# matuszelenak/Hybrid-Genome-Assembler

Hardware: AMD Instinct MI355X
Metric: k-mers/s counted + reads/s categorized, k=19 E.coli 30×; %HBM roofline (higher is better)
Workload: dtype u64; 1 GPU; C2: k=19 count of an E. coli-sized pair (4.64 + 5.07 Mb, d=0.021), ART-like 30x 150 bp, 2 files; per step: count_run + spec_hist + select[10,25]; k=19, reads=1941478, bases=293163176, instances_per_gpu=256275096, distinct_rows=6680801, selected=1820729, discriminative=1820245, buckets=4096, max_split=1, parallelism=dp1

## Files before the change

### hybrid-genome-assembler_amd/csrc/api.hip

```cpp
#include <cstdlib>
#include <cstring>
#include <string>
#include <type_traits>
#include <vector>

#include "hga_internal.hpp"

namespace {
thread_local std::string g_err;

template <class F>
hga_status guard(F&& f) {
    static_assert(std::is_void<decltype(f())>::value, "guarded bodies return nothing");
    try {
        g_err.clear();
        f();
        return HGA_OK;
    } catch (const hga::Error& e) {
        g_err = e.what();
        return e.code;
    } catch (const std::bad_alloc&) {
        g_err = "host allocation failed";
        return HGA_ERR_OOM;
    } catch (const std::exception& e) {
// ... 51 lines not shown
        HGA_REQUIRE(device >= 0 && device < nd, HGA_ERR_INVALID, "no such HIP device");
        HGA_HIP(hipSetDevice(device));
        auto* c = new hga_ctx();
        c->device = device;
        hipDeviceProp_t prop;
        if (hipGetDeviceProperties(&prop, device) == hipSuccess && prop.multiProcessorCount > 0)
            c->num_cu = prop.multiProcessorCount;
        hipError_t e = hipStreamCreateWithFlags(&c->stream, hipStreamNonBlocking);
        if (e != hipSuccess) {
            delete c;
            throw hga::Error(HGA_ERR_HIP, std::string("hipStreamCreate: ") + hipGetErrorString(e));
        }
        *out = c;
    });
}

hga_status hga_ctx_destroy(hga_ctx* c) {
    if (!c) return HGA_OK;
    return guard([&] {
        (void)hipSetDevice(c->device);
        (void)hipStreamSynchronize(c->stream);
        if (c->side) (void)hipStreamSynchronize(c->side);
        hipStream_t s = c->stream, s2 = c->side;
        hipEvent_t e1 = c->ev_fork, e2 = c->ev_join;
        delete c;
        (void)hipStreamDestroy(s);
        if (s2) {
            (void)hipEventDestroy(e1);
            (void)hipEventDestroy(e2);
            (void)hipStreamDestroy(s2);
        }
    });
}

hga_status hga_count_begin(hga_ctx* c, int k, uint32_t n_files) {
    HGA_CTX_GUARD(c, hga::count_begin(c, k, n_files));
}

hga_status hga_count_add(hga_ctx* c, uint32_t file, const char* seq, uint64_t n_bytes) {
    HGA_CTX_GUARD(c, {
        HGA_REQUIRE(seq || n_bytes == 0, HGA_ERR_INVALID, "null sequence pointer");
        hga::count_add(c, file, seq, n_bytes);
    });
}

hga_status hga_connections_run(hga_ctx* c, const uint32_t* pivots, uint64_t n_pivots, uint32_t min_kmers,
                               uint64_t min_score, const int32_t* categories, uint64_t* n) {
    HGA_CTX_GUARD(c, {
// ... 384 lines not shown
```

### hybrid-genome-assembler_amd/csrc/count.hip

```cpp
#include <algorithm>
#include <cstdlib>
#include <cstring>
#include <map>
#include <type_traits>

#include "hga_internal.hpp"
#include "kmer_dev.hpp"

#ifndef HGA_B1_NOFB
#define HGA_B1_NOFB 0
#endif
#ifndef HGA_B1_BRANCHFREE
#define HGA_B1_BRANCHFREE 0
#endif

namespace hga {
namespace {

constexpr int NT_B = 512;
constexpr int P_B = 16;
constexpr int TP_B = NT_B * P_B;
constexpr uint64_t ST_ALIGN = TP_B;
#ifndef HGA_MAX_FB
#define HGA_MAX_FB 12
// ... 561 lines not shown
    }
    __syncthreads();
#pragma unroll
    for (int j = 0; j < IT; ++j) {
        const uint32_t i = (uint32_t)j * NT_R + tid;
        if (i < used) stage[off2[dd[j]] + rk[j]] = ee[j];
    }
    __syncthreads();
    for (uint32_t d = (uint32_t)__builtin_amdgcn_readfirstlane(tid >> 6); d < nb2; d += NT_R / 64) {
        const uint32_t o = off2[d], len = off2[d + 1] - o;
        E* __restrict__ dst = out + base2[d];
        for (uint32_t jj = (uint32_t)(tid & 63); jj < len; jj += 64) {
            if (HGA_NT_REBIN_ST) __builtin_nontemporal_store(stage[o + jj], &dst[jj]);
            else dst[jj] = stage[o + jj];
        }
    }
}

template <class E1, class E>
__global__ void __launch_bounds__(NT_R_MAX) kc_rebin(const E1* __restrict__ in1, const Blk* __restrict__ table,
                                                 const unsigned long long* __restrict__ gstat, uint32_t W,
                                                 KP kp, const uint32_t* __restrict__ nblk,
                                                 unsigned long long* __restrict__ off,
                                                 E* __restrict__ out, bool first) {
    if (first) {
        rebin_block<E1, E>(blockIdx.x, in1, table, W, kp, nblk, off, out);
        return;
    }
    const uint64_t n_first = (uint64_t)W * kp.nb1, used = gstat[3];
    for (uint64_t blk = n_first + blockIdx.x; blk < used; blk += gridDim.x) {
        rebin_block<E1, E>(blk, in1, table, W, kp, nblk, off, out);
        __syncthreads();
    }
}

#ifndef HGA_GROUP
#define HGA_GROUP 4
#endif
constexpr int GRP = HGA_GROUP;
template <class E>
__device__ __forceinline__ void read_group(const E* keys, uint32_t g, E (&k)[GRP]) {
    if constexpr (sizeof(E) == 4) {
#pragma unroll
        for (int t = 0; t < GRP / 4; ++t) {
            const uint4 v = reinterpret_cast<const uint4*>(keys)[g * (GRP / 4) + t];
            k[4 * t] = v.x; k[4 * t + 1] = v.y; k[4 * t + 2] = v.z; k[4 * t + 3] = v.w;
        }
    } else {
#pragma unroll
        for (int t = 0; t < GRP / 2; ++t) {
            const ulonglong2 a = reinterpret_cast<const ulonglong2*>(keys)[g * (GRP / 2) + t];
            k[2 * t] = a.x; k[2 * t + 1] = a.y;
        }
// ... 1117 lines not shown
    };
    if (lo > hi) {
        if (t < 4) span[t] = 0;
        publish(0u);
        return;
    }
    uint32_t lg = 0;
    while ((hi >> lg) - (lo >> lg) + 1 > 256) ++lg;
    const uint32_t dbase = lo >> lg;
    uint32_t sum = 0;
    const uint32_t b0 = (dbase + t) << lg;
    for (uint32_t b = b0; b < b0 + (1u << lg); ++b)
        if (b >= lo && b <= hi) sum += hist[b];
    if (t == 0) {
        span[0] = lo;
        span[1] = hi;
        span[2] = lg;
        span[3] = dbase;
    }
    publish(sum);
}

constexpr uint32_t BX_MAX = 1024;
__global__ void __launch_bounds__(1024) kc_bx_prep(const uint32_t* __restrict__ hist, const unsigned long long* __restrict__ wcnt,
                                                   uint32_t grid, uint32_t* __restrict__ dbase,
                                                   unsigned long long* __restrict__ stat,
                                                   unsigned long long* __restrict__ hstat) {
    __shared__ uint32_t ws[1024 / 64 + 1];
    __shared__ unsigned long long red[3][16];
    const uint32_t t = threadIdx.x, lane = t & 63, wave = t >> 6;
    uint32_t h[4], sum = 0, mx = 0;
#pragma unroll
    for (int q = 0; q < 4; ++q) {
        h[q] = hist[4 * t + q];
        sum += h[q];
        mx = max(mx, h[q]);
    }
    uint32_t tot;
    uint32_t o = block_excl_scan<1024>(sum, ws, &tot);
#pragma unroll
    for (int q = 0; q < 4; ++q) {
        dbase[4 * t + q] = o;
        o += h[q];
    }
    unsigned long long k = 0, d = 0, m = mx;
    for (uint32_t i = t; i < grid; i += 1024) {
        k += wcnt[2 * i];
        d += wcnt[2 * i + 1];
    }
#pragma unroll
    for (int s2 = 32; s2; s2 >>= 1) {
        k += __shfl_xor(k, s2, 64);
        d += __shfl_xor(d, s2, 64);
        m = max(m, (unsigned long long)__shfl_xor(m, s2, 64));
    }
    if (lane == 0) {
        red[0][wave] = k;
        red[1][wave] = d;
        red[2][wave] = m;
    }
    __syncthreads();
    if (t < 4) {
        unsigned long long v = 0;
        for (int w = 0; w < 16; ++w) v = t == 2 ? max(v, red[2][w]) : v + (t < 2 ? red[t][w] : 0ull);
        stat[t] = v;
        hstat[t] = v;
    }
}
__global__ void __launch_bounds__(256) kc_bx_colscan(const uint32_t* __restrict__ rows, uint32_t n_rows,
                                                     const uint32_t* __restrict__ dbase, uint32_t* __restrict__ off) {
    __shared__ uint32_t part[16][17];
    const uint32_t dl = threadIdx.x & 15, rg = threadIdx.x >> 4, d = blockIdx.x * 16 + dl;
    const uint32_t per = (n_rows + 15) / 16, r0 = rg * per, r1 = min(n_rows, r0 + per);
    uint32_t s2 = 0;
    for (uint32_t r = r0; r < r1; ++r) s2 += rows[(uint64_t)r * SEL_HB + d];
    part[rg][dl] = s2;
    __syncthreads();
    uint32_t base = dbase[d];
    for (uint32_t g = 0; g < rg; ++g) base += part[g][dl];
    for (uint32_t r = r0; r < r1; ++r) {
        off[(uint64_t)r * SEL_HB + d] = base;
        base += rows[(uint64_t)r * SEL_HB + d];
    }
}
__global__ void __launch_bounds__(256) kc_bx_scatter(const uint64_t* __restrict__ wkeys, uint64_t region,
                                                     const unsigned long long* __restrict__ wcnt,
                                                     const uint32_t* __restrict__ off, int hshift,
                                                     uint64_t* __restrict__ out) {
    __shared__ uint32_t cur[SEL_HB];
    const uint32_t w = blockIdx.x;
    for (uint32_t i = threadIdx.x; i < SEL_HB; i += 256) cur[i] = off[(uint64_t)w * SEL_HB + i];
    __syncthreads();
    const uint64_t n = wcnt[2 * w];
    const uint64_t* __restrict__ src = wkeys + (uint64_t)w * region;
    for (uint64_t j = threadIdx.x; j < n; j += 256) {
        const uint64_t key = src[j];
        const uint32_t pos = atomicAdd(&cur[(uint32_t)(key >> hshift) & (SEL_HB - 1)], 1u);
        out[pos] = key;
    }
}
template <int R>
__device__ __forceinline__ void bx_sort_seg(uint64_t* __restrict__ keys, uint32_t start, uint32_t len, uint32_t lane,
                                            int bits) {
    const uint64_t cm = bits >= 63 ? ~0ull >> 1 : (1ull << bits) - 1;
    uint64_t v[R];
#pragma unroll
    for (int u = 0; u < R; ++u) {
        const uint32_t i = lane * R + u;
        const uint64_t k = i < len ? keys[start + i] : 0ull;
        v[u] = i < len ? ((k & cm) << 1) | (k >> 63) : ~0ull;
    }
    bitonic_stage<R, 2>(v, lane);
// ... 4 lines not shown
    }
}
template <int R>
__device__ __forceinline__ void bx_sort_seg32(uint64_t* __restrict__ keys, uint32_t start, uint32_t len, uint32_t lane,
                                              int bits, uint64_t dig) {
    const int lb = bits - 12;
    const uint64_t lm = (1ull << lb) - 1;
    uint32_t v[R];
#pragma unroll
    for (int u = 0; u < R; ++u) {
        const uint32_t i = lane * R + u;
        const uint64_t k = i < len ? keys[start + i] : 0ull;
        v[u] = i < len ? (uint32_t)(((k & lm) << 1) | (k >> 63)) : ~0u;
    }
    bitonic_stage<R, 2>(v, lane);
    const uint64_t hi = dig << lb;
#pragma unroll
    for (int u = 0; u < R; ++u) {
        const uint32_t i = lane * R + u;
        if (i < len) keys[start + i] = hi | (uint64_t)(v[u] >> 1) | ((uint64_t)(v[u] & 1u) << 63);
    }
}
__global__ void __launch_bounds__(256) kc_bx_wsort(uint64_t* __restrict__ keys, const uint32_t* __restrict__ hist,
                                                   const uint32_t* __restrict__ dbase, int bits) {
    const uint32_t d = blockIdx.x * 4 + (threadIdx.x >> 6), lane = threadIdx.x & 63;
    const uint32_t len = hist[d], st = dbase[d];
    if (len <= 1 || len > BX_MAX) return;
    if (bits - 12 + 1 <= 32) {
        if (len <= 64) bx_sort_seg32<1>(keys, st, len, lane, bits, d);
        else if (len <= 256) bx_sort_seg32<4>(keys, st, len, lane, bits, d);
        else if (len <= 512) bx_sort_seg32<8>(keys, st, len, lane, bits, d);
        else bx_sort_seg32<16>(keys, st, len, lane, bits, d);
        return;
    }
    if (len <= 64) bx_sort_seg<1>(keys, st, len, lane, bits);
    else if (len <= 256) bx_sort_seg<4>(keys, st, len, lane, bits);
    else if (len <= 512) bx_sort_seg<8>(keys, st, len, lane, bits);
    else bx_sort_seg<16>(keys, st, len, lane, bits);
}

constexpr uint32_t BX_CAP32 = SS_T * 2 * SS_I;
template <bool U32, int NT, int I, int DB>
__global__ void __launch_bounds__(NT) kc_bx_lsort(uint64_t* __restrict__ keys, const uint32_t* __restrict__ hist,
                                                  const uint32_t* __restrict__ dbase, int bits, uint32_t min_len) {
    using T = std::conditional_t<U32, uint32_t, uint64_t>;
    __shared__ T sk[NT * I];
    __shared__ uint32_t wcnt[NT / 64][1 << DB];
// ... 195 lines not shown

    uint64_t st_pos = total_bytes / ((uint64_t)c->num_cu * HGA_B1_PER_CU) + 1;
    const uint64_t st_cap = (uint64_t)BLK * nb1 * 15 / 16;
    const char* sole_env = std::getenv("HGA_B1_SOLE");
    if ((!sole_env || std::atoi(sole_env) != 0) && st_pos > st_cap + st_cap / 2) st_pos = st_cap;
    st_pos = std::max<uint64_t>(ST_ALIGN, (st_pos + ST_ALIGN - 1) / ST_ALIGN * ST_ALIGN);
    std::vector<uint32_t> n_st(F, 0);
    std::vector<BinFile> bf(F);
    uint32_t W = 0;
    for (uint32_t f = 0; f < F; ++f) {
        n_st[f] = (uint32_t)((s.seq_len[f] + st_pos - 1) / st_pos);
        bf[f].n = s.seq_len[f];
        bf[f].w0 = W;
        W += n_st[f];
    }

    auto* gstat = static_cast<unsigned long long*>(s.cursor.ensure(8 * 8));
    uint64_t* fs = static_cast<uint64_t*>(s.file_start.ensure((size_t)nb * (F + 1) * 8));
    uint32_t* wcnt = static_cast<uint32_t*>(s.fine_hist.ensure((size_t)std::max<uint32_t>(W, 1) * nb * 4));
    auto* off = static_cast<unsigned long long*>(s.cursor2.ensure(((size_t)W * nb + 1) * 8));
    uint32_t* nblk = static_cast<uint32_t*>(s.nblk.ensure((size_t)std::max<uint32_t>(W, 1) * nb1 * 4));
    for (uint32_t f = 0; f < F; ++f) bf[f].seq = s.seq[f]->as<uint8_t>();
    const size_t tb = sizeof(BinFile) * F;
    std::vector<char> tab(tb);
    std::memcpy(tab.data(), bf.data(), tb);
    char* d_tab = static_cast<char*>(s.bin_files.ensure(tb));
    if (s.tab_host != tab) {
        HGA_HIP(hipMemcpy(d_tab, tab.data(), tb, hipMemcpyHostToDevice));
        s.tab_host = tab;
    }
    BinFile* d_bf = reinterpret_cast<BinFile*>(d_tab);

    const size_t esz1 = e1_32 ? 4 : 8, esz = e32 ? 4 : 8;
    uint64_t cap = (total_bytes / std::max<uint32_t>(1, min_per_file) + 4) & ~3ull;
    if (const char* e = std::getenv("HGA_ROW_CAP")) cap = std::max<uint64_t>(4, std::strtoull(e, nullptr, 10) & ~3ull);
    const uint32_t slot_b = (uint32_t)esz + 4u * F;
    uint32_t T = 1;
    while ((uint64_t)T * 2 * slot_b <= LDS_TAB) T *= 2;
    HGA_REQUIRE(T >= 2 * NT_C, HGA_ERR_INVALID, "too many files for the LDS table");
    const uint32_t maxload = std::min<uint32_t>((uint32_t)(T * 0.85), T - NT_C - 8);
    void* binned = s.binned.ensure(std::max<size_t>(total_bytes, 1) * esz);

    const uint64_t n_first = (uint64_t)W * nb1;
    const uint64_t table_cap = n_first + total_bytes / BLK + 2;
    const uint64_t pool_cap = table_cap * BLK;
    void* binned1 = s.binned1.ensure(pool_cap * esz1);
    Blk* table = static_cast<Blk*>(s.regions.ensure(table_cap * sizeof(Blk)));
    c->launch("kc_init", [&] { hipLaunchKernelGGL(kc_init_stat, dim3(1), dim3(64), 0, c->stream, gstat, n_first); });
    c->check_launch("kc_init");

    if (W) {
        c->launch("kc_bin1", [&] {
#define HGA_BIN1(E1T, KK, FBB)                                                                              \
    hipLaunchKernelGGL((kc_bin1<E1T, KK, FBB>), dim3(W), dim3(NT_B), 0, c->stream, d_bf, F, st_pos, kp, table, table_cap, \
                       pool_cap, static_cast<E1T*>(binned1), wcnt, nblk, gstat)
            if (e1_32 && kp.k == 19 && kp.fb == MAX_FB && !HGA_B1_NOFB) HGA_BIN1(uint32_t, 19, MAX_FB);
            else if (e1_32 && kp.k == 19) HGA_BIN1(uint32_t, 19, 0);
            else if (e1_32 && kp.k == 17) HGA_BIN1(uint32_t, 17, 0);
            else if (e1_32 && kp.k == 15) HGA_BIN1(uint32_t, 15, 0);
            else if (e1_32) HGA_BIN1(uint32_t, 0, 0);
            else if (kp.k == 21) HGA_BIN1(uint64_t, 21, 0);
            else HGA_BIN1(uint64_t, 0, 0);
#undef HGA_BIN1
        });
        c->check_launch("kc_bin1");
    }
    c->launch("kc_layout", [&] {
        hipLaunchKernelGGL(kc_transpose, dim3(blocks_for(nb, 64), blocks_for(std::max<uint32_t>(W, 1), 64)), dim3(256),
                           0, c->stream, wcnt, W, nb, reinterpret_cast<uint64_t*>(off));
    });
    c->check_launch("kc_transpose");
    exclusive_scan_u64(c, reinterpret_cast<uint64_t*>(off), (uint64_t)W * nb + 1, s.scratch);
    c->launch("kc_layout", [&] {
        hipLaunchKernelGGL(kc_fs, dim3(blocks_for((uint64_t)nb * (F + 1), 256)), dim3(256), 0, c->stream,
                           reinterpret_cast<const uint64_t*>(off), d_bf, W, nb, F, fs);
    });
    c->check_launch("kc_fs");
    const unsigned spill_grid = (unsigned)std::min<uint64_t>(table_cap - n_first, HGA_SPILL_GRID);
    c->launch("kc_rebin", [&] {
#define HGA_REBIN(E1T, ET)                                                                                 \
    do {                                                                                                   \
        if (n_first)                                                                                       \
            hipLaunchKernelGGL((kc_rebin<E1T, ET>), dim3((unsigned)n_first), dim3(rebin_nt<ET>()), 0, c->stream, \
                               static_cast<const E1T*>(binned1), table, gstat, W, kp, nblk, off,            \
                               static_cast<ET*>(binned), true);                                              \
        if (spill_grid)                                                                                    \
            hipLaunchKernelGGL((kc_rebin<E1T, ET>), dim3(spill_grid), dim3(rebin_nt<ET>()), 0, c->stream,  \
                               static_cast<const E1T*>(binned1), table, gstat, W, kp, nblk, off,            \
                               static_cast<ET*>(binned), false);                                             \
    } while (0)
        if (e1_32 && e32) HGA_REBIN(uint32_t, uint32_t);
        else if (e32) HGA_REBIN(uint64_t, uint32_t);
        else if (e1_32) HGA_REBIN(uint32_t, uint64_t);
        else HGA_REBIN(uint64_t, uint64_t);
#undef HGA_REBIN
    });
    c->check_launch("kc_rebin");
    uint32_t fb3 = 0;
    {
        const uint64_t avg = total_bytes >> fb;
        const char* te = std::getenv("HGA_SPLIT3_TARGET");
        const char* fe = std::getenv("HGA_SPLIT3_FORCE");
        const uint64_t target = te ? std::strtoull(te, nullptr, 10) : 32768;
        if (fe) {
            const uint32_t want = (uint32_t)std::atoi(fe);
            while (fb3 < want && fb3 < 8 && ((2u << fb3) * F) <= MAX_SF3 && kp.rbits - fb3 > 1) ++fb3;
        } else if (avg > 2 * per_bucket && fb == MAX_FB) {
            while (fb3 < 8 && (avg >> fb3) > target && ((2u << fb3) * F) <= MAX_SF3 && kp.rbits - fb3 > 10) ++fb3;
        }
    }
    if (fb3) {
        const uint32_t S = 1u << fb3;
        void* binned3 = s.binned3.ensure((total_bytes + total_bytes / 4 + (uint64_t)nb * S * SLACK_3 + 64) * esz);
// ... 222 lines not shown
    const bool use_bnd = n_thr <= 8 && !std::getenv("HGA_SPEC_FP64");
    if (fresh || s.thr_dev != thr) {
        HGA_HIP(hipMemcpyAsync(dthr, hthr, n_thr * 8, hipMemcpyHostToDevice, c->stream));
        if (n_thr <= 8) {
            std::vector<uint16_t> b((size_t)TL * 8, 0xFFFF);
            for (uint32_t t = 1; t < TL; ++t)
                for (uint32_t i = 0; i < n_thr; ++i) {
                    uint32_t lo = 0, hi = t + 1;
                    while (lo < hi) {
                        const uint32_t mid = (lo + hi) / 2;
                        const volatile double x = (double)mid / (double)t;
                        if (thr[i] <= x * 100.0) hi = mid; else lo = mid + 1;
                    }
                    b[(size_t)t * 8 + i] = lo > t ? 0xFFFF : (uint16_t)lo;
                }
            HGA_HIP(hipMemcpy(dbnd, b.data(), b.size() * 2, hipMemcpyHostToDevice));
        }
        s.thr_dev = thr;
    }
    const bool pend = s.pending;
    const uint64_t rows_hint = pend ? s.rows_cap : s.rows;
    const unsigned grid = (unsigned)std::min<uint64_t>(blocks_for(std::max<uint64_t>((rows_hint + 3) / 4, 1), NT_S * SG_S),
                                                       (uint64_t)c->num_cu);
    c->launch("kc_spec_hist", [&] {
        hipLaunchKernelGGL(kc_spec_hist, dim3(grid), dim3(NT_S), (size_t)n_thr * TL * 4, c->stream,
                           s.rows_cnt.as<uint32_t>(), rows_hint,
                           pend ? static_cast<const unsigned long long*>(s.cursor.p) : nullptr, s.rows_cap, s.n_files,
                           dthr, n_thr, use_bnd ? (const uint4*)dbnd : nullptr,
                           hist, over, ctrl, over_cap);
    });
    c->check_launch("kc_spec_hist");
    const uint64_t ncap = 1u << 20;
    auto* comp = static_cast<unsigned long long*>(s.hist_comp.ensure(ncap * 16 + 64));
    const uint64_t nd = (uint64_t)n_thr * TD;
    c->launch("kc_spec_hist", [&] {
        hipLaunchKernelGGL(kc_hist_compact, dim3(blocks_for(nd, NT_HC)), dim3(NT_HC), 0, c->stream, hist, n_thr, comp,
                           ctrl, ncap, c->pinned.dev(hcomp), SPEC_CHUNK);
        if (before_publish) (*before_publish)(ctrl, comp);
        hipLaunchKernelGGL(kc_spec_publish, dim3(1), dim3(64), 0, c->stream, ctrl,
                           pend ? static_cast<const unsigned long long*>(s.cursor.p) : nullptr, c->pinned.dev(hc),
                           c->pinned.dev(hrun));
    });
    c->check_launch("kc_hist_compact");
    c->sync();
    s.last_err = 0;
    if (pend) count_settle(c, hrun);
    s.last_err = ((hc[1] & 1ull) ? 8ull : 0ull) | ((hc[1] & 2ull) ? 16ull : 0ull) | (hc[2] > ncap ? 32ull : 0ull);
    HGA_REQUIRE(!(hc[1] & 1ull), HGA_ERR_INVALID, "a row's specificity is above the last threshold");
    HGA_REQUIRE(!(hc[1] & 2ull), HGA_ERR_OOM, "histogram overflow list full");
    HGA_REQUIRE(hc[2] <= ncap, HGA_ERR_OOM, "histogram compaction buffer full");
    std::vector<std::pair<uint64_t, uint64_t>> bins;
    bins.reserve(hc[2] + std::min<uint64_t>(hc[0], over_cap));
    if (hc[2]) {
        const unsigned long long* cv = hcomp;
        std::vector<unsigned long long> rest;
        if (hc[2] > SPEC_CHUNK) {
            rest.resize(2 * hc[2]);
            HGA_HIP(hipMemcpy(rest.data(), comp, hc[2] * 16, hipMemcpyDeviceToHost));
            cv = rest.data();
        }
        for (uint64_t i = 0; i < hc[2]; ++i) bins.emplace_back(cv[2 * i], cv[2 * i + 1]);
    }
    if (hc[0]) {
// ... 36 lines not shown
    }
    const uint32_t sel_grid = s.rows < (1ull << 25) && !std::getenv("HGA_SEL_GRID_X") ? std::min(s.sel_grid, 512u)
                                                                                        : s.sel_grid;
    const uint32_t cpw = (uint32_t)blocks_for(chunks, sel_grid);
    const unsigned grid = (unsigned)blocks_for(chunks, cpw);
    const uint64_t region = (uint64_t)cpw * NT_H * SEL_R;
    const size_t hb = (size_t)SEL_HB * 4;
    const size_t rows_b = msd ? (size_t)grid * hb : 0;
    char* tb = static_cast<char*>(s.sel_tmp.ensure(64 + hb + 1024 + rows_b + (size_t)grid * 16 + (msd ? hb + rows_b : 0)));
    auto* wcnt = reinterpret_cast<unsigned long long*>(tb + 64 + hb + 1024 + rows_b);
    uint32_t* bx_dbase = msd ? reinterpret_cast<uint32_t*>(tb + 64 + hb + 1024 + rows_b + (size_t)grid * 16) : nullptr;
    uint32_t* bx_off = msd ? bx_dbase + SEL_HB : nullptr;
    char* wt = static_cast<char*>(s.sel_wtmp.ensure((size_t)grid * region * (flag_bit ? 8 : 12) + 64));
    uint64_t* wkeys = reinterpret_cast<uint64_t*>(wt);
    uint32_t* wflag = reinterpret_cast<uint32_t*>(wt + (size_t)grid * region * 8);
    auto* stat = reinterpret_cast<unsigned long long*>(tb);
    uint32_t* dhist = reinterpret_cast<uint32_t*>(tb + 64);
    uint32_t* dig256 = reinterpret_cast<uint32_t*>(tb + 64 + hb);
    uint32_t* dhist_rows = msd ? reinterpret_cast<uint32_t*>(tb + 64 + hb + 1024) : nullptr;
    char* hp = static_cast<char*>(c->pinned_sel.ensure(64 + 1024));
    auto* hs = reinterpret_cast<unsigned long long*>(hp);
    uint32_t* h256 = reinterpret_cast<uint32_t*>(hp + 64);
    if (!s.rows) HGA_HIP(hipMemsetAsync(stat, 0, 64, c->stream));
    if (s.rows) {
        c->launch("kc_select", [&] {
            hipLaunchKernelGGL(kc_select, dim3(grid), dim3(NT_H), 0, c->stream, s.rows_key.as<uint64_t>(),
                               s.rows_cnt.as<uint32_t>(), s.rows, s.rows_cap, s.n_files, lower, upper, wkeys, wflag,
                               flag_bit, cpw, wcnt, dhist_rows, bits - 12, stat, msd ? dhist : nullptr);
            if (msd) {
                hipLaunchKernelGGL(kc_dhist_reduce, dim3(SEL_HB / 256, (grid + 31) / 32), dim3(256), 0, c->stream,
                                   dhist_rows, grid, dhist);
                hipLaunchKernelGGL(kc_bx_prep, dim3(1), dim3(1024), 0, c->stream, (const uint32_t*)dhist,
                                   (const unsigned long long*)wcnt, grid, bx_dbase, stat, c->pinned_sel.dev(hs));
            } else {
                hipLaunchKernelGGL(kc_sel_compact, dim3(grid), dim3(256), 0, c->stream, (const uint64_t*)wkeys,
                                   (const uint32_t*)wflag, region, (const unsigned long long*)wcnt, grid, out, flag,
                                   flag_bit, stat);
            }
        });
        c->check_launch("kc_select");
    }
    if (!(s.rows && msd)) HGA_HIP(hipMemcpyAsync(hs, stat, 64, hipMemcpyDeviceToHost, c->stream));
    if (before_sync) (*before_sync)(stat);
    c->sync();
    const uint64_t n = hs[0];
    const bool u32seg = bits - 12 + 1 <= 32;
    const bool bx = msd && n > 1 && hs[2] <= (u32seg ? (uint64_t)BX_CAP32 : (uint64_t)SS_CAP) && !std::getenv("HGA_BX_OFF");
    if (bx) {
        c->launch("bx_colscan", [&] {
            hipLaunchKernelGGL(kc_bx_colscan, dim3(SEL_HB / 16), dim3(256), 0, c->stream, (const uint32_t*)dhist_rows,
                               grid, (const uint32_t*)bx_dbase, bx_off);
        });
        c->launch("bx_scatter", [&] {
            hipLaunchKernelGGL(kc_bx_scatter, dim3(grid), dim3(256), 0, c->stream, (const uint64_t*)wkeys, region,
                               (const unsigned long long*)wcnt, (const uint32_t*)bx_off, bits - 12, out);
        });
        c->launch("radix_segsort", [&] {
            hipLaunchKernelGGL(kc_bx_wsort, dim3(SEL_HB / 4), dim3(256), 0, c->stream, out, (const uint32_t*)dhist,
                               (const uint32_t*)bx_dbase, bits);
        });
        c->check_launch("kc_bx_wsort");
        if (hs[2] > BX_MAX) {
            c->launch("radix_segsort", [&] {
                if (u32seg && !std::getenv("HGA_BX_LSD")) {
                    hipLaunchKernelGGL(kc_bx_csort, dim3(SEL_HB), dim3(CS_T), 0, c->stream, out, (const uint32_t*)dhist,
                                       (const uint32_t*)bx_dbase, bits, BX_MAX);
                } else if (u32seg) {
                    hipLaunchKernelGGL((kc_bx_lsort<true, 512, 32, 9>), dim3(SEL_HB), dim3(512), 0, c->stream, out,
                                       (const uint32_t*)dhist, (const uint32_t*)bx_dbase, bits, BX_MAX);
                    if (hs[2] > 16384u)
                        hipLaunchKernelGGL((kc_bx_lsort<true, 1024, 32, 8>), dim3(SEL_HB), dim3(1024), 0, c->stream,
                                           out, (const uint32_t*)dhist, (const uint32_t*)bx_dbase, bits, 16384u);
                } else {
                    hipLaunchKernelGGL((kc_bx_lsort<false, SS_T, SS_I, 8>), dim3(SEL_HB), dim3(SS_T), 0, c->stream,
                                       out, (const uint32_t*)dhist, (const uint32_t*)bx_dbase, bits, BX_MAX);
                }
            });
            c->check_launch("kc_bx_lsort");
        }
    } else if (msd && n > 1) {
        c->launch("kc_select", [&] {
            hipLaunchKernelGGL(kc_sel_compact, dim3(grid), dim3(256), 0, c->stream, (const uint64_t*)wkeys,
                               (const uint32_t*)wflag, region, (const unsigned long long*)wcnt, grid, out, flag,
                               flag_bit, stat);
// ... 145 lines not shown
```

### hybrid-genome-assembler_amd/csrc/hga_internal.hpp

```cpp
#pragma once

#include <hip/hip_runtime.h>

#include <cstdint>
#include <cstring>
#include <algorithm>
#include <map>
#include <memory>
#include <stdexcept>
#include <string>
#include <unordered_map>
#include <functional>
#include <vector>

#include "../../include/hga.h"

namespace hga {

struct Error : std::runtime_error {
    hga_status code;
    Error(hga_status c, const std::string& m) : std::runtime_error(m), code(c) {}
};

#define HGA_HIP(call)                                                                      \
// ... 185 lines not shown
struct TailsState {
    DevBuf ex, ey, et, lx, ly, ov, tptr, key, val, sort, where, twin, head, pos, rp, link_a, link_b, w, part, flag_l,
        flag_r, tmax, tfar, far_id, ptr_l, ptr_r, out_l, out_r;
};

struct Comm {
    int rank = 0, nranks = 1;
    int root = -1;
    DevBuf stage;
    PinnedBuf hstage;
    virtual ~Comm() = default;
    virtual bool on_device() const = 0;
    virtual void alltoallv(hga_ctx* c, const void* const* send, const uint64_t* send_bytes, void* const* recv,
                           const uint64_t* recv_bytes) = 0;
};

}

struct hga_ctx {
    int device = 0;
    hipStream_t stream = nullptr;
    hipStream_t side = nullptr;
    hipEvent_t ev_fork = nullptr, ev_join = nullptr;
    hipStream_t side_stream() {
        if (!side) {
            HGA_HIP(hipStreamCreateWithFlags(&side, hipStreamNonBlocking));
            HGA_HIP(hipEventCreateWithFlags(&ev_fork, hipEventDisableTiming));
            HGA_HIP(hipEventCreateWithFlags(&ev_join, hipEventDisableTiming));
        }
        return side;
    }
    int num_cu = 256;
    hga::Profiler prof;
    hga::CountState count;
    hga::LookupState lookup;
    hga::ConnState conn;
    hga::OverlapState overlap;
    hga::ComponentState comp;
    hga::TailsState tails;
    hga::PinnedBuf pinned;
    hga::PinnedBuf pinned_sel;
    std::unique_ptr<hga::Comm> comm;
    hga::DevBuf scan_state;
    uint64_t scan_tiles = 0;
    uint32_t scan_epoch = 0;

// ... 97 lines not shown
void count_rows_to(hga_ctx* c, uint64_t** keys, uint32_t** counts, uint64_t* n_rows);
void count_rows_device(hga_ctx* c, DevBuf& keys, DevBuf& counts);
void count_rows_global(hga_ctx* c, int file, std::vector<uint64_t>& keys, std::vector<uint32_t>& counts);
void lookup_gather(hga_ctx* c);
void connections_gather(hga_ctx* c, uint64_t* n);

void lookup_load(hga_ctx* c, int k, const uint64_t* keys, uint32_t n);
void lookup_set_reads(hga_ctx* c, const char* bases, const uint64_t* offsets, uint64_t n,
                      uint32_t first_id);
void lookup_run(hga_ctx* c);
void lookup_pack(hga_ctx* c, bool skip_codes = false);
void lookup_sizes(hga_ctx* c, hga_lookup_sizes* out);
void lookup_fetch(hga_ctx* c, const hga_lookup_result* out);
void hll_registers(hga_ctx* c, int k, int b, uint8_t* regs);

void radix_sort_u64(hga_ctx* c, uint64_t* keys, uint32_t* vals, uint64_t n, int bits,
                    DevBuf& scratch);
void radix_sort_u64_from(hga_ctx* c, const uint64_t* src_k, uint64_t* keys, uint64_t n, int bits, DevBuf& scratch);
void radix_sort_u32(hga_ctx* c, uint32_t* keys, uint32_t* vals, uint64_t n, int bits,
                    DevBuf& scratch);
void radix_sort_u32_from(hga_ctx* c, const uint32_t* src_k, const uint32_t* src_v, uint32_t* keys, uint32_t* vals,
                         uint64_t n, int bits, DevBuf& scratch);
void exclusive_scan_u64(hga_ctx* c, uint64_t* data, uint64_t n, DevBuf& scratch);
struct ScanTicket {
    unsigned long long* status;
    unsigned long long* ctr;
    uint64_t tbase;
    uint32_t epoch;
};
ScanTicket scan_ticket(hga_ctx* c, uint64_t nt);
void count_settle(hga_ctx* c, const unsigned long long* h = nullptr);
void count_dense(hga_ctx* c);
bool segment_sort(hga_ctx* c, const uint64_t* hptr, uint64_t nseg, uint64_t maxlen, int kbits, uint64_t* sk,
                  uint32_t* sv, DevBuf& list_buf, unsigned long long* ctr2, const char* label,
                  uint32_t* lists = nullptr, const unsigned long long* lists_n = nullptr);
void sort_export_u64(hga_ctx* c, uint64_t* keys, uint64_t n, int shift, uint32_t dbase, const uint32_t* d_hist,
                     const uint32_t* h_hist, DevBuf& scratch);
}
```

### hybrid-genome-assembler_amd/csrc/sort.hip

```cpp
#include <algorithm>
#include <cstdlib>

#include "hga_internal.hpp"
#include "kmer_dev.hpp"

namespace hga {
namespace {

constexpr int RS_T = 256;
#ifndef HGA_RS_I
#define HGA_RS_I 16
#endif
constexpr int RS_I = HGA_RS_I;
constexpr int RS_TILE = RS_T * RS_I;
constexpr int SC_T = 1024, SC_I = 4, SC_TILE = SC_T * SC_I;
#ifndef HGA_RS_MAX_DIGIT
#define HGA_RS_MAX_DIGIT 10
#endif
#ifndef HGA_LBW
#define HGA_LBW 8
#endif

template <class K, int DB>
__global__ void __launch_bounds__(RS_T) rs_upsweep(const K* __restrict__ keys, uint64_t n,
// ... 298 lines not shown
#pragma unroll
    for (int j = 0; j < SC_I; ++j) {
        v[j] = base + j < n ? (uint64_t)data[base + j] : 0ull;
        sum += v[j];
    }
    const uint64_t inc = wave_incl_scan64(sum, lane);
    if (lane == 63) ws[wave] = inc;
    __syncthreads();
    if (threadIdx.x == 0) {
        uint64_t agg = 0;
        for (int w = 0; w < SC_T / 64; ++w) {
            const uint64_t x = ws[w];
            ws[w] = agg;
            agg += x;
        }
        s_pre = chained_lookback(status, tile, agg, epoch);
    }
    __syncthreads();
    uint64_t run = s_pre + ws[wave] + inc - sum;
#pragma unroll
    for (int j = 0; j < SC_I; ++j) {
        if (base + j < n) data[base + j] = (T)run;
        run += v[j];
    }
}

}

ScanTicket scan_ticket(hga_ctx* c, uint64_t nt) {
    const size_t need = 256 + nt * 8;
    const bool fresh = need > c->scan_state.cap;
    auto* st = static_cast<unsigned long long*>(c->scan_state.ensure(std::max<size_t>(need, 1 << 16)));
    if (fresh) {
        HGA_HIP(hipMemsetAsync(st, 0, c->scan_state.cap, c->stream));
        c->scan_tiles = 0;
    }
    if (++c->scan_epoch == SCS_EPOCHS) {
        HGA_HIP(hipMemsetAsync(st + 32, 0, c->scan_state.cap - 256, c->stream));
        c->scan_epoch = 1;
    }
    ScanTicket t{st + 32, st, c->scan_tiles, c->scan_epoch};
    c->scan_tiles += nt;
    return t;
}

namespace {
// ... 199 lines not shown
            if (shift > 0) radix_sort_u64(c, k2 + st, nullptr, h_hist[d], shift, tmp);
            HGA_HIP(hipMemcpyAsync(keys + st, k2 + st, (size_t)h_hist[d] * 8, hipMemcpyDeviceToDevice, c->stream));
            c->sync();
        }
        st += h_hist[d];
    }
}
void radix_sort_u64_from(hga_ctx* c, const uint64_t* src_k, uint64_t* keys, uint64_t n, int bits, DevBuf& scratch) {
    radix_sort_impl<uint64_t>(c, keys, nullptr, n, bits, scratch, src_k, nullptr);
}
void radix_sort_u32(hga_ctx* c, uint32_t* keys, uint32_t* vals, uint64_t n, int bits,
                    DevBuf& scratch) {
    radix_sort_impl<uint32_t>(c, keys, vals, n, bits > 32 ? 32 : bits, scratch);
}
void radix_sort_u32_from(hga_ctx* c, const uint32_t* src_k, const uint32_t* src_v, uint32_t* keys, uint32_t* vals,
                         uint64_t n, int bits, DevBuf& scratch) {
    radix_sort_impl<uint32_t>(c, keys, vals, n, bits > 32 ? 32 : bits, scratch, src_k, src_v);
}
void exclusive_scan_u64(hga_ctx* c, uint64_t* data, uint64_t n, DevBuf& scratch) {
    (void)scratch;
    excl_scan_impl<uint64_t>(c, data, n);
}

}
```

Before: 173.8 billion k-mers/s.

## Fuse layout transpose/scan/fs, merge rebin launches, and speculate bx select path

Replaces the transpose + exclusive scan + kc_fs sequence with a single decoupled-lookback kernel that reads the count matrix transposed into shared memory and writes file splits directly. Merges the two kc_rebin launches into one grid whose later blocks handle spill work. In select, folds bx_prep into a templated colscan and launches scatter/wsort speculatively before the host sync, gated by a device-side go flag, and waits on an event instead of a full stream sync. The aim is fewer launches and less host round-trip latency, at the cost of redundant per-block prep work and kernels that may launch only to exit early.

```diff
diff --git a/hybrid-genome-assembler_amd/csrc/api.hip b/hybrid-genome-assembler_amd/csrc/api.hip
--- a/hybrid-genome-assembler_amd/csrc/api.hip
+++ b/hybrid-genome-assembler_amd/csrc/api.hip
@@ -97,8 +97,9 @@
         (void)hipStreamSynchronize(c->stream);
         if (c->side) (void)hipStreamSynchronize(c->side);
         hipStream_t s = c->stream, s2 = c->side;
-        hipEvent_t e1 = c->ev_fork, e2 = c->ev_join;
+        hipEvent_t e1 = c->ev_fork, e2 = c->ev_join, e3 = c->ev_sel;
         delete c;
+        if (e3) (void)hipEventDestroy(e3);
         (void)hipStreamDestroy(s);
         if (s2) {
             (void)hipEventDestroy(e1);
diff --git a/hybrid-genome-assembler_amd/csrc/count.hip b/hybrid-genome-assembler_amd/csrc/count.hip
--- a/hybrid-genome-assembler_amd/csrc/count.hip
+++ b/hybrid-genome-assembler_amd/csrc/count.hip
@@ -607,13 +607,14 @@
                                                  const unsigned long long* __restrict__ gstat, uint32_t W,
                                                  KP kp, const uint32_t* __restrict__ nblk,
                                                  unsigned long long* __restrict__ off,
-                                                 E* __restrict__ out, bool first) {
-    if (first) {
+                                                 E* __restrict__ out) {
+    const uint64_t n_first = (uint64_t)W * kp.nb1;
+    if (blockIdx.x < n_first) {
         rebin_block<E1, E>(blockIdx.x, in1, table, W, kp, nblk, off, out);
         return;
     }
-    const uint64_t n_first = (uint64_t)W * kp.nb1, used = gstat[3];
-    for (uint64_t blk = n_first + blockIdx.x; blk < used; blk += gridDim.x) {
+    const uint64_t used = gstat[3], stride = gridDim.x - n_first;
+    for (uint64_t blk = (uint64_t)blockIdx.x; blk < used; blk += stride) {
         rebin_block<E1, E>(blk, in1, table, W, kp, nblk, off, out);
         __syncthreads();
     }
@@ -1777,10 +1778,12 @@
 }
 
 constexpr uint32_t BX_MAX = 1024;
+constexpr uint32_t BX_GO = 6;
+__host__ __device__ inline bool bx_go(uint64_t n, uint64_t m, uint64_t go_cap) { return n > 1 && m <= go_cap; }
 __global__ void __launch_bounds__(1024) kc_bx_prep(const uint32_t* __restrict__ hist, const unsigned long long* __restrict__ wcnt,
                                                    uint32_t grid, uint32_t* __restrict__ dbase,
                                                    unsigned long long* __restrict__ stat,
-                                                   unsigned long long* __restrict__ hstat) {
+                                                   unsigned long long* __restrict__ hstat, uint64_t go_cap) {
     __shared__ uint32_t ws[1024 / 64 + 1];
     __shared__ unsigned long long red[3][16];
     const uint32_t t = threadIdx.x, lane = t & 63, wave = t >> 6;
@@ -1821,17 +1824,88 @@
         stat[t] = v;
         hstat[t] = v;
     }
-}
+    if (t == 0) {
+        unsigned long long n = 0, m = 0;
+        for (int w = 0; w < 16; ++w) {
+            n += red[0][w];
+            m = max(m, red[2][w]);
+        }
+        stat[BX_GO] = bx_go(n, m, go_cap) ? 1ull : 0ull;
+    }
+}
+template <bool PREP>
 __global__ void __launch_bounds__(256) kc_bx_colscan(const uint32_t* __restrict__ rows, uint32_t n_rows,
-                                                     const uint32_t* __restrict__ dbase, uint32_t* __restrict__ off) {
+                                                     uint32_t* __restrict__ dbase, uint32_t* __restrict__ off,
+                                                     unsigned long long* __restrict__ stat,
+                                                     const uint32_t* __restrict__ hist,
+                                                     const unsigned long long* __restrict__ wcnt,
+                                                     unsigned long long* __restrict__ hstat, uint64_t go_cap) {
     __shared__ uint32_t part[16][17];
+    __shared__ uint32_t s_db[16];
+    if constexpr (PREP) {
+        static_assert(SEL_HB == 256 * 16, "one thread per 16 digit totals");
+        __shared__ uint32_t ws[256 / 64 + 1];
+        __shared__ uint32_t s_mx[4];
+        __shared__ unsigned long long red[2][4];
+        const uint32_t t = threadIdx.x, lane = t & 63, wave = t >> 6;
+        uint32_t h[16], sum = 0, mx = 0;
+#pragma unroll
+        for (int q = 0; q < 4; ++q) {
+            const uint4 v = reinterpret_cast<const uint4*>(hist)[4 * t + q];
+            h[4 * q] = v.x; h[4 * q + 1] = v.y; h[4 * q + 2] = v.z; h[4 * q + 3] = v.w;
+        }
+#pragma unroll
+        for (int q = 0; q < 16; ++q) {
+            sum += h[q];
+            mx = max(mx, h[q]);
+        }
+        uint32_t tot;
+        uint32_t o = block_excl_scan<256>(sum, ws, &tot);
+        if (t == blockIdx.x) {
+#pragma unroll
+            for (int q = 0; q < 16; ++q) {
+                s_db[q] = o;
+                dbase[16 * t + q] = o;
+                o += h[q];
+            }
+        }
+        unsigned long long k = 0, dc = 0;
+        if (blockIdx.x == 0)
+            for (uint32_t i = t; i < n_rows; i += 256) {
+                k += wcnt[2 * i];
+                dc += wcnt[2 * i + 1];
+            }
+#pragma unroll
+        for (int s2 = 32; s2; s2 >>= 1) {
+            mx = max(mx, (uint32_t)__shfl_xor(mx, s2, 64));
+            k += __shfl_xor(k, s2, 64);
+            dc += __shfl_xor(dc, s2, 64);
+        }
+        if (lane == 0) {
+            s_mx[wave] = mx;
+            red[0][wave] = k;
+            red[1][wave] = dc;
+        }
+        __syncthreads();
+        const uint32_t m = max(max(s_mx[0], s_mx[1]), max(s_mx[2], s_mx[3]));
+        const bool go = bx_go(tot, m, go_cap);
+        if (blockIdx.x == 0 && t < 4) {
+            const unsigned long long v = t == 2 ? m : t < 2 ? red[t][0] + red[t][1] + red[t][2] + red[t][3] : 0ull;
+            stat[t] = v;
+            hstat[t] = v;
+            if (t == 0) stat[BX_GO] = go ? 1ull : 0ull;
+        }
+        if (!go) return;
+    } else {
+        if (!stat[BX_GO]) return;
+    }
     const uint32_t dl = threadIdx.x & 15, rg = threadIdx.x >> 4, d = blockIdx.x * 16 + dl;
     const uint32_t per = (n_rows + 15) / 16, r0 = rg * per, r1 = min(n_rows, r0 + per);
     uint32_t s2 = 0;
     for (uint32_t r = r0; r < r1; ++r) s2 += rows[(uint64_t)r * SEL_HB + d];
     part[rg][dl] = s2;
     __syncthreads();
-    uint32_t base = dbase[d];
+    uint32_t base = PREP ? s_db[dl] : dbase[d];
     for (uint32_t g = 0; g < rg; ++g) base += part[g][dl];
     for (uint32_t r = r0; r < r1; ++r) {
         off[(uint64_t)r * SEL_HB + d] = base;
@@ -1841,8 +1915,10 @@
 __global__ void __launch_bounds__(256) kc_bx_scatter(const uint64_t* __restrict__ wkeys, uint64_t region,
                                                      const unsigned long long* __restrict__ wcnt,
                                                      const uint32_t* __restrict__ off, int hshift,
-                                                     uint64_t* __restrict__ out) {
+                                                     uint64_t* __restrict__ out,
+                                                     const unsigned long long* __restrict__ stat) {
     __shared__ uint32_t cur[SEL_HB];
+    if (!stat[BX_GO]) return;
     const uint32_t w = blockIdx.x;
     for (uint32_t i = threadIdx.x; i < SEL_HB; i += 256) cur[i] = off[(uint64_t)w * SEL_HB + i];
     __syncthreads();
@@ -1893,7 +1969,9 @@
     }
 }
 __global__ void __launch_bounds__(256) kc_bx_wsort(uint64_t* __restrict__ keys, const uint32_t* __restrict__ hist,
-                                                   const uint32_t* __restrict__ dbase, int bits) {
+                                                   const uint32_t* __restrict__ dbase, int bits,
+                                                   const unsigned long long* __restrict__ stat) {
+    if (!stat[BX_GO]) return;
     const uint32_t d = blockIdx.x * 4 + (threadIdx.x >> 6), lane = threadIdx.x & 63;
     const uint32_t len = hist[d], st = dbase[d];
     if (len <= 1 || len > BX_MAX) return;
@@ -2135,14 +2213,16 @@
     uint32_t* nblk = static_cast<uint32_t*>(s.nblk.ensure((size_t)std::max<uint32_t>(W, 1) * nb1 * 4));
     for (uint32_t f = 0; f < F; ++f) bf[f].seq = s.seq[f]->as<uint8_t>();
     const size_t tb = sizeof(BinFile) * F;
-    std::vector<char> tab(tb);
+    std::vector<char> tab(tb + 4 * (size_t)F);
     std::memcpy(tab.data(), bf.data(), tb);
-    char* d_tab = static_cast<char*>(s.bin_files.ensure(tb));
+    for (uint32_t f = 0; f < F; ++f) std::memcpy(tab.data() + tb + 4 * (size_t)f, &bf[f].w0, 4);
+    char* d_tab = static_cast<char*>(s.bin_files.ensure(tab.size()));
     if (s.tab_host != tab) {
-        HGA_HIP(hipMemcpy(d_tab, tab.data(), tb, hipMemcpyHostToDevice));
+        HGA_HIP(hipMemcpy(d_tab, tab.data(), tab.size(), hipMemcpyHostToDevice));
         s.tab_host = tab;
     }
     BinFile* d_bf = reinterpret_cast<BinFile*>(d_tab);
+    const uint32_t* d_w0 = reinterpret_cast<const uint32_t*>(d_tab + tb);
 
     const size_t esz1 = e1_32 ? 4 : 8, esz = e32 ? 4 : 8;
     uint64_t cap = (total_bytes / std::max<uint32_t>(1, min_per_file) + 4) & ~3ull;
@@ -2178,30 +2258,26 @@
         });
         c->check_launch("kc_bin1");
     }
-    c->launch("kc_layout", [&] {
-        hipLaunchKernelGGL(kc_transpose, dim3(blocks_for(nb, 64), blocks_for(std::max<uint32_t>(W, 1), 64)), dim3(256),
-                           0, c->stream, wcnt, W, nb, reinterpret_cast<uint64_t*>(off));
-    });
-    c->check_launch("kc_transpose");
-    exclusive_scan_u64(c, reinterpret_cast<uint64_t*>(off), (uint64_t)W * nb + 1, s.scratch);
-    c->launch("kc_layout", [&] {
-        hipLaunchKernelGGL(kc_fs, dim3(blocks_for((uint64_t)nb * (F + 1), 256)), dim3(256), 0, c->stream,
-                           reinterpret_cast<const uint64_t*>(off), d_bf, W, nb, F, fs);
-    });
-    c->check_launch("kc_fs");
+    if (std::getenv("HGA_LAYOUT_T") ||
+        !layout_scan(c, wcnt, W, nb, reinterpret_cast<uint64_t*>(off), d_w0, F, fs)) {
+        c->launch("kc_layout", [&] {
+            hipLaunchKernelGGL(kc_transpose, dim3(blocks_for(nb, 64), blocks_for(std::max<uint32_t>(W, 1), 64)),
+                               dim3(256), 0, c->stream, wcnt, W, nb, reinterpret_cast<uint64_t*>(off));
+        });
+        c->check_launch("kc_transpose");
+        exclusive_scan_u64(c, reinterpret_cast<uint64_t*>(off), (uint64_t)W * nb + 1, s.scratch);
+        c->launch("kc_layout", [&] {
+            hipLaunchKernelGGL(kc_fs, dim3(blocks_for((uint64_t)nb * (F + 1), 256)), dim3(256), 0, c->stream,
+                               reinterpret_cast<const uint64_t*>(off), d_bf, W, nb, F, fs);
+        });
+        c->check_launch("kc_fs");
+    }
     const unsigned spill_grid = (unsigned)std::min<uint64_t>(table_cap - n_first, HGA_SPILL_GRID);
     c->launch("kc_rebin", [&] {
 #define HGA_REBIN(E1T, ET)                                                                                 \
-    do {                                                                                                   \
-        if (n_first)                                                                                       \
-            hipLaunchKernelGGL((kc_rebin<E1T, ET>), dim3((unsigned)n_first), dim3(rebin_nt<ET>()), 0, c->stream, \
-                               static_cast<const E1T*>(binned1), table, gstat, W, kp, nblk, off,            \
-                               static_cast<ET*>(binned), true);                                              \
-        if (spill_grid)                                                                                    \
-            hipLaunchKernelGGL((kc_rebin<E1T, ET>), dim3(spill_grid), dim3(rebin_nt<ET>()), 0, c->stream,  \
-                               static_cast<const E1T*>(binned1), table, gstat, W, kp, nblk, off,            \
-                               static_cast<ET*>(binned), false);                                             \
-    } while (0)
+    hipLaunchKernelGGL((kc_rebin<E1T, ET>), dim3((unsigned)n_first + spill_grid), dim3(rebin_nt<ET>()), 0,  \
+                       c->stream, static_cast<const E1T*>(binned1), table, gstat, W, kp, nblk, off,        \
+                       static_cast<ET*>(binned))
         if (e1_32 && e32) HGA_REBIN(uint32_t, uint32_t);
         else if (e32) HGA_REBIN(uint64_t, uint32_t);
         else if (e1_32) HGA_REBIN(uint32_t, uint64_t);
@@ -2470,10 +2546,10 @@
     const uint64_t rows_hint = pend ? s.rows_cap : s.rows;
     const unsigned grid = (unsigned)std::min<uint64_t>(blocks_for(std::max<uint64_t>((rows_hint + 3) / 4, 1), NT_S * SG_S),
                                                        (uint64_t)c->num_cu);
+    const unsigned long long* run = pend ? static_cast<const unsigned long long*>(s.cursor.p) : nullptr;
     c->launch("kc_spec_hist", [&] {
         hipLaunchKernelGGL(kc_spec_hist, dim3(grid), dim3(NT_S), (size_t)n_thr * TL * 4, c->stream,
-                           s.rows_cnt.as<uint32_t>(), rows_hint,
-                           pend ? static_cast<const unsigned long long*>(s.cursor.p) : nullptr, s.rows_cap, s.n_files,
+                           s.rows_cnt.as<uint32_t>(), rows_hint, run, s.rows_cap, s.n_files,
                            dthr, n_thr, use_bnd ? (const uint4*)dbnd : nullptr,
                            hist, over, ctrl, over_cap);
     });
@@ -2485,8 +2561,7 @@
         hipLaunchKernelGGL(kc_hist_compact, dim3(blocks_for(nd, NT_HC)), dim3(NT_HC), 0, c->stream, hist, n_thr, comp,
                            ctrl, ncap, c->pinned.dev(hcomp), SPEC_CHUNK);
         if (before_publish) (*before_publish)(ctrl, comp);
-        hipLaunchKernelGGL(kc_spec_publish, dim3(1), dim3(64), 0, c->stream, ctrl,
-                           pend ? static_cast<const unsigned long long*>(s.cursor.p) : nullptr, c->pinned.dev(hc),
+        hipLaunchKernelGGL(kc_spec_publish, dim3(1), dim3(64), 0, c->stream, ctrl, run, c->pinned.dev(hc),
                            c->pinned.dev(hrun));
     });
     c->check_launch("kc_hist_compact");
@@ -2569,6 +2644,38 @@
     auto* hs = reinterpret_cast<unsigned long long*>(hp);
     uint32_t* h256 = reinterpret_cast<uint32_t*>(hp + 64);
     if (!s.rows) HGA_HIP(hipMemsetAsync(stat, 0, 64, c->stream));
+    const bool u32seg = bits - 12 + 1 <= 32;
+    const bool bx_on = !std::getenv("HGA_BX_OFF");
+    const uint64_t go_cap = bx_on ? (u32seg ? (uint64_t)BX_CAP32 : (uint64_t)SS_CAP) : 0ull;
+    const bool spec = s.rows && msd && bx_on && !before_sync;
+    bool ev_counts = false;
+    auto bx_front = [&](bool prep) {
+        c->launch("bx_colscan", [&] {
+            if (prep)
+                hipLaunchKernelGGL(kc_bx_colscan<true>, dim3(SEL_HB / 16), dim3(256), 0, c->stream,
+                                   (const uint32_t*)dhist_rows, grid, bx_dbase, bx_off, stat, (const uint32_t*)dhist,
+                                   (const unsigned long long*)wcnt, c->pinned_sel.dev(hs), go_cap);
+            else
+                hipLaunchKernelGGL(kc_bx_colscan<false>, dim3(SEL_HB / 16), dim3(256), 0, c->stream,
+                                   (const uint32_t*)dhist_rows, grid, bx_dbase, bx_off, stat, (const uint32_t*)dhist,
+                                   (const unsigned long long*)wcnt, c->pinned_sel.dev(hs), go_cap);
+        });
+        if (prep) {
+            if (!c->ev_sel) HGA_HIP(hipEventCreateWithFlags(&c->ev_sel, hipEventDisableTiming));
+            HGA_HIP(hipEventRecord(c->ev_sel, c->stream));
+            ev_counts = true;
+        }
+        c->launch("bx_scatter", [&] {
+            hipLaunchKernelGGL(kc_bx_scatter, dim3(grid), dim3(256), 0, c->stream, (const uint64_t*)wkeys, region,
+                               (const unsigned long long*)wcnt, (const uint32_t*)bx_off, bits - 12, out,
+                               (const unsigned long long*)stat);
+        });
+        c->launch("radix_segsort", [&] {
+            hipLaunchKernelGGL(kc_bx_wsort, dim3(SEL_HB / 4), dim3(256), 0, c->stream, out, (const uint32_t*)dhist,
+                               (const uint32_t*)bx_dbase, bits, (const unsigned long long*)stat);
+        });
+        c->check_launch("kc_bx_wsort");
+    };
     if (s.rows) {
         c->launch("kc_select", [&] {
             hipLaunchKernelGGL(kc_select, dim3(grid), dim3(NT_H), 0, c->stream, s.rows_key.as<uint64_t>(),
@@ -2577,8 +2684,10 @@
             if (msd) {
                 hipLaunchKernelGGL(kc_dhist_reduce, dim3(SEL_HB / 256, (grid + 31) / 32), dim3(256), 0, c->stream,
                                    dhist_rows, grid, dhist);
-                hipLaunchKernelGGL(kc_bx_prep, dim3(1), dim3(1024), 0, c->stream, (const uint32_t*)dhist,
-                                   (const unsigned long long*)wcnt, grid, bx_dbase, stat, c->pinned_sel.dev(hs));
+                if (!spec)
+                    hipLaunchKernelGGL(kc_bx_prep, dim3(1), dim3(1024), 0, c->stream, (const uint32_t*)dhist,
+                                       (const unsigned long long*)wcnt, grid, bx_dbase, stat, c->pinned_sel.dev(hs),
+                                       go_cap);
             } else {
                 hipLaunchKernelGGL(kc_sel_compact, dim3(grid), dim3(256), 0, c->stream, (const uint64_t*)wkeys,
                                    (const uint32_t*)wflag, region, (const unsigned long long*)wcnt, grid, out, flag,
@@ -2586,27 +2695,19 @@
             }
         });
         c->check_launch("kc_select");
+        if (spec) bx_front(true);
     }
     if (!(s.rows && msd)) HGA_HIP(hipMemcpyAsync(hs, stat, 64, hipMemcpyDeviceToHost, c->stream));
     if (before_sync) (*before_sync)(stat);
-    c->sync();
+    if (ev_counts) {
+        HGA_HIP(hipEventSynchronize(c->ev_sel));
+    } else {
+        c->sync();
+    }
     const uint64_t n = hs[0];
-    const bool u32seg = bits - 12 + 1 <= 32;
-    const bool bx = msd && n > 1 && hs[2] <= (u32seg ? (uint64_t)BX_CAP32 : (uint64_t)SS_CAP) && !std::getenv("HGA_BX_OFF");
+    const bool bx = msd && bx_go(n, hs[2], go_cap);
     if (bx) {
-        c->launch("bx_colscan", [&] {
-            hipLaunchKernelGGL(kc_bx_colscan, dim3(SEL_HB / 16), dim3(256), 0, c->stream, (const uint32_t*)dhist_rows,
-                               grid, (const uint32_t*)bx_dbase, bx_off);
-        });
-        c->launch("bx_scatter", [&] {
-            hipLaunchKernelGGL(kc_bx_scatter, dim3(grid), dim3(256), 0, c->stream, (const uint64_t*)wkeys, region,
-                               (const unsigned long long*)wcnt, (const uint32_t*)bx_off, bits - 12, out);
-        });
-        c->launch("radix_segsort", [&] {
-            hipLaunchKernelGGL(kc_bx_wsort, dim3(SEL_HB / 4), dim3(256), 0, c->stream, out, (const uint32_t*)dhist,
-                               (const uint32_t*)bx_dbase, bits);
-        });
-        c->check_launch("kc_bx_wsort");
+        if (!spec) bx_front(false);
         if (hs[2] > BX_MAX) {
             c->launch("radix_segsort", [&] {
                 if (u32seg && !std::getenv("HGA_BX_LSD")) {
diff --git a/hybrid-genome-assembler_amd/csrc/hga_internal.hpp b/hybrid-genome-assembler_amd/csrc/hga_internal.hpp
--- a/hybrid-genome-assembler_amd/csrc/hga_internal.hpp
+++ b/hybrid-genome-assembler_amd/csrc/hga_internal.hpp
@@ -231,6 +231,7 @@
     hipStream_t stream = nullptr;
     hipStream_t side = nullptr;
     hipEvent_t ev_fork = nullptr, ev_join = nullptr;
+    hipEvent_t ev_sel = nullptr;
     hipStream_t side_stream() {
         if (!side) {
             HGA_HIP(hipStreamCreateWithFlags(&side, hipStreamNonBlocking));
@@ -374,6 +375,8 @@
 void radix_sort_u32_from(hga_ctx* c, const uint32_t* src_k, const uint32_t* src_v, uint32_t* keys, uint32_t* vals,
                          uint64_t n, int bits, DevBuf& scratch);
 void exclusive_scan_u64(hga_ctx* c, uint64_t* data, uint64_t n, DevBuf& scratch);
+bool layout_scan(hga_ctx* c, const uint32_t* wcnt, uint32_t W, uint32_t nb, uint64_t* off, const uint32_t* w0,
+                 uint32_t F, uint64_t* fs);
 struct ScanTicket {
     unsigned long long* status;
     unsigned long long* ctr;
diff --git a/hybrid-genome-assembler_amd/csrc/sort.hip b/hybrid-genome-assembler_amd/csrc/sort.hip
--- a/hybrid-genome-assembler_amd/csrc/sort.hip
+++ b/hybrid-genome-assembler_amd/csrc/sort.hip
@@ -344,6 +344,74 @@
     for (int j = 0; j < SC_I; ++j) {
         if (base + j < n) data[base + j] = (T)run;
         run += v[j];
+    }
+}
+
+__global__ void __launch_bounds__(SC_T) sc_layout(const uint32_t* __restrict__ wcnt, uint32_t W, uint32_t nb,
+                                                  uint64_t* __restrict__ off, const uint32_t* __restrict__ w0,
+                                                  uint32_t F, uint64_t* __restrict__ fs,
+                                                  unsigned long long* __restrict__ status,
+                                                  unsigned long long* __restrict__ ctr, uint64_t tbase, uint32_t epoch) {
+    __shared__ uint64_t ws[SC_T / 64];
+    __shared__ uint64_t s_tile, s_pre;
+    __shared__ uint32_t tv[SC_TILE];
+    __shared__ uint64_t sv[SC_TILE];
+    const int lane = threadIdx.x & 63, wave = threadIdx.x >> 6;
+    if (threadIdx.x == 0) s_tile = atomicAdd(ctr, 1ull) - tbase;
+    for (uint32_t l = threadIdx.x; l < (uint32_t)SC_TILE; l += SC_T) tv[l] = 0;
+    __syncthreads();
+    const uint64_t tile = s_tile;
+    const uint64_t n = (uint64_t)W * nb + 1;
+    const uint64_t i0 = tile * SC_TILE, i1 = i0 + SC_TILE < n ? i0 + SC_TILE : n;
+    const uint64_t ne = i1 < n - 1 ? i1 : n - 1;
+    const uint32_t b_lo = (uint32_t)(i0 / W);
+    if (ne > i0) {
+        const uint32_t nbk = (uint32_t)((ne - 1) / W) - b_lo + 1;
+        const uint32_t np = W * nbk;
+        for (uint32_t p = threadIdx.x; p < np; p += SC_T) {
+            const uint32_t w = p / nbk, b = b_lo + (p - w * nbk);
+            const uint64_t i = (uint64_t)b * W + w;
+            if (i >= i0 && i < ne) tv[i - i0] = wcnt[(uint64_t)w * nb + b];
+        }
+    }
+    __syncthreads();
+    const uint32_t lb = threadIdx.x * SC_I;
+    uint64_t v[SC_I];
+    uint64_t sum = 0;
+#pragma unroll
+    for (int j = 0; j < SC_I; ++j) {
+        v[j] = tv[lb + j];
+        sum += v[j];
+    }
+    const uint64_t inc = wave_incl_scan64(sum, lane);
+    if (lane == 63) ws[wave] = inc;
+    __syncthreads();
+    if (threadIdx.x == 0) {
+        uint64_t agg = 0;
+        for (int w = 0; w < SC_T / 64; ++w) {
+            const uint64_t x = ws[w];
+            ws[w] = agg;
+            agg += x;
+        }
+        s_pre = chained_lookback(status, tile, agg, epoch);
+    }
+    __syncthreads();
+    uint64_t run = s_pre + ws[wave] + inc - sum;
+#pragma unroll
+    for (int j = 0; j < SC_I; ++j) {
+        if (i0 + lb + j < n) off[i0 + lb + j] = run;
+        sv[lb + j] = run;
+        run += v[j];
+    }
+    __syncthreads();
+    const uint32_t bs = b_lo ? b_lo - 1 : 0;
+    const uint64_t bl = (i1 - 1) / W;
+    const uint32_t be = bl < nb ? (uint32_t)bl : nb - 1;
+    const uint32_t nc = (be - bs + 1) * (F + 1);
+    for (uint32_t q = threadIdx.x; q < nc; q += SC_T) {
+        const uint32_t b = bs + q / (F + 1), f = q % (F + 1);
+        const uint64_t idx = f == F ? (uint64_t)(b + 1) * W : (uint64_t)b * W + w0[f];
+        if (idx >= i0 && idx < i1) fs[(uint64_t)b * (F + 1) + f] = sv[idx - i0];
     }
 }
 
@@ -589,4 +657,19 @@
     excl_scan_impl<uint64_t>(c, data, n);
 }
 
-}
+bool layout_scan(hga_ctx* c, const uint32_t* wcnt, uint32_t W, uint32_t nb, uint64_t* off, const uint32_t* w0,
+                 uint32_t F, uint64_t* fs) {
+    constexpr uint32_t LAYOUT_W_MAX = SC_TILE / 4;
+    if (W == 0 || W > LAYOUT_W_MAX) return false;
+    const uint64_t n = (uint64_t)W * nb + 1;
+    const uint64_t nt = (n + SC_TILE - 1) / SC_TILE;
+    const ScanTicket t = scan_ticket(c, nt);
+    c->launch("kc_layout", [&] {
+        hipLaunchKernelGGL(sc_layout, dim3((unsigned)nt), dim3(SC_T), 0, c->stream, wcnt, W, nb, off, w0, F, fs,
+                           t.status, t.ctr, t.tbase, t.epoch);
+    });
+    c->check_launch("sc_layout");
+    return true;
+}
+
+}
```

Result: faster. 177.3 billion k-mers/s, median of 6 (+2.0%).
